# JanBeh/radiorust

Measured on NVIDIA B200. Metric: complex MS/s via FreqShift->Filter->Downsampler, higher is better.
Workload: dtype f32

## Files before the change

### radiorust_b200/csrc/rr_fused.cu

```cuda
#include <cuda.h>
#include <cuda_runtime.h>

#include <algorithm>
#include <cstdio>
#include <cstdlib>
#include <mutex>

#include "rr_kernels.h"
#include "rr_poly.cuh"
#include "rr_pk.cuh"

namespace rr {

namespace {

constexpr int FK = 512;
constexpr int FRK = 10;
constexpr int T_WARPS = FRK / 2;
constexpr int T_THREADS = 32 * T_WARPS;
constexpr int F_ROWS = 32;
constexpr int PITCH = FRK * 8;
constexpr int STAGE_ROWS = 528;
constexpr int STAGE_BYTES = STAGE_ROWS * PITCH;
constexpr int TW_UNITS = 17;
// ... 28 lines not shown
        : "memory");
}
__device__ __forceinline__ void mb_wait_long(uint32_t bar, uint32_t parity) {
    asm volatile(
        "{\n"
        ".reg .pred p;\n"
        "LWAIT_%=:\n"
        "mbarrier.try_wait.parity.acquire.cta.shared::cta.b64 p, [%0], %1, %2;\n"
        "@p bra LDONE_%=;\n"
        "bra LWAIT_%=;\n"
        "LDONE_%=:\n"
        "}\n" ::"r"(bar),
        "r"(parity), "r"(20000u)
        : "memory");
}
__device__ __forceinline__ pc f_lds(uint32_t addr) {
    pc r;
    asm volatile("ld.shared.v2.f32 {%0, %1}, [%2];" : "=f"(r.x), "=f"(r.y) : "r"(addr));
    return r;
}
__device__ __forceinline__ void f_lds2(uint32_t addr, pc& a, pc& b) {
    asm volatile("ld.shared.v4.f32 {%0, %1, %2, %3}, [%4];" : "=f"(a.x), "=f"(a.y), "=f"(b.x), "=f"(b.y) : "r"(addr));
}
__device__ __forceinline__ void f_sts(uint32_t addr, pc a) {
    asm volatile("st.shared.v2.f32 [%0], {%1, %2};" ::"r"(addr), "f"(a.x), "f"(a.y) : "memory");
}
__device__ __forceinline__ void f_sts2(uint32_t addr, pc a, pc b) {
    asm volatile("st.shared.v4.f32 [%0], {%1, %2, %3, %4};" ::"r"(addr), "f"(a.x), "f"(a.y), "f"(b.x), "f"(b.y) : "memory");
}
__device__ __forceinline__ void f_ldg2(const float4* p, pc& a, pc& b) {
    asm volatile("ld.global.nc.v4.f32 {%0, %1, %2, %3}, [%4];" : "=f"(a.x), "=f"(a.y), "=f"(b.x), "=f"(b.y) : "l"(p));
}

__device__ __forceinline__ pc f_rotation(uint32_t d, uint32_t numer_abs, uint32_t denom, double inv_m, int sign) {
    const uint32_t r = mulmod_fast(numer_abs, d % denom, denom, inv_m);
    double s, c;
    sincospi(2.0 * (double)r / (double)denom, &s, &c);
    return pc((float)c, (float)(sign < 0 ? -s : s));
}

__device__ __forceinline__ void f_pass1_store(pc (&v)[32], uint32_t tw_row, uint32_t xch_wr) {
    pdft_regs<32, +1>(v);
    pc w[3][2];
    f_lds2(tw_row, w[0][0], w[0][1]);
    f_lds2(tw_row + 16, w[1][0], w[1][1]);
#pragma unroll
    for (int m = 0; m < 16; ++m) {
        if (m + 2 < 16) f_lds2(tw_row + (m + 2) * 16, w[(m + 2) % 3][0], w[(m + 2) % 3][1]);
        f_sts(xch_wr + (2 * m) * PITCH, pcmul(v[2 * m], w[m % 3][0]));
        f_sts(xch_wr + (2 * m + 1) * PITCH, pcmul(v[2 * m + 1], w[m % 3][1]));
    }
}

#ifdef RR_FUSED_PROF
#define PROF(...) __VA_ARGS__
__device__ long long g_fused_prof[256 * 16];
#else
#define PROF(...)
#endif

struct FusedGeom {
    int steps, S0, hp, slot_bytes, slot_stride;
};
__host__ __device__ inline FusedGeom fused_geom(int P) {
    FusedGeom g;
    g.steps = P / 2;
    g.S0 = (g.steps + 1) / 2;
    g.hp = 2 * g.S0 + ((g.S0 & 1) ? 0 : 2);
    if (g.hp > P) g.hp = P;
    g.slot_bytes = F_ROWS * g.hp * 8;
    g.slot_stride = (g.slot_bytes + 127) / 128 * 128;
    return g;
}

template <int S_LO, int S_HI, bool HAS_NCO>
__device__ __forceinline__ void f_steps(pc (&acc)[FRK], const float4* __restrict__ xrow, const float4* __restrict__ crow, const float4* cf_base) {
#pragma unroll
    for (int st = S_LO; st < S_HI; ++st) {
        const float4 xv = xrow[st];
        pc x0(xv.x, xv.y), x1(xv.z, xv.w);
        if (HAS_NCO) {
            const float4 cv = crow[st];
            x0 = pcmul(x0, pc(cv.x, cv.y));
            x1 = pcmul(x1, pc(cv.z, cv.w));
        }
        const float4* cf = cf_base + st * 5;
        const float4 a0 = cf[0], a1 = cf[1], a2 = cf[2], a3 = cf[3], a4 = cf[4];
        const float k0[FRK] = {a0.x, a0.y, a0.z, a0.w, a1.x, a1.y, a1.z, a1.w, a2.x, a2.y};
        const float k1[FRK] = {a2.z, a2.w, a3.x, a3.y, a3.z, a3.w, a4.x, a4.y, a4.z, a4.w};
#pragma unroll
        for (int c = 0; c < FRK; ++c) {
            acc[c] = pfma_s(x0, k0[c], acc[c]);
            acc[c] = pfma_s(x1, k1[c], acc[c]);
        }
    }
}

}

template <int FW, int D, int NB, bool HAS_NCO, int PT>
__global__ void __launch_bounds__(T_THREADS + 32 * FW, 1)
k_fused(const __grid_constant__ CUtensorMap tmap, const FusedArgs a, const int n_streams) {
    extern __shared__ __align__(128) unsigned char smem[];
    const int warp = __shfl_sync(0xffffffffu, (int)(threadIdx.x >> 5), 0), lane = threadIdx.x & 31;
    const int P = PT > 0 ? PT : a.P;
    const FusedGeom geo = fused_geom(P);
    const int Lmax = a.Lmax, V = a.V, n_out = a.n_out;
    const int B = (n_out + V - 1) / V;
    const int n_tiles = (B * V + F_ROWS - 1) / F_ROWS;

    const int keep_bytes = ((Lmax * PITCH) + 127) / 128 * 128;
    unsigned char* const p_stage = smem;
    unsigned char* const p_tw = p_stage + 2 * STAGE_BYTES;
    unsigned char* const p_keep = p_tw + TW_BYTES;
    unsigned char* const p_ys = p_keep + keep_bytes;
    unsigned char* const p_ring = p_ys + (((size_t)NB * YS_STRIDE * 8 + 127) / 128 * 128);
    unsigned char* const p_colph = p_ring + (size_t)FW * D * geo.slot_stride;
    unsigned char* const p_bar = p_colph + (((size_t)FW * P * 8 + 127) / 128 * 128);
    const uint32_t bar_full = s_u32(p_bar), bar_empty = bar_full + 16, bar_ring = bar_full + 32;
    const uint32_t left_cnt = bar_ring + FW * D * 8;

    for (int e = threadIdx.x; e < 2 * STAGE_BYTES / 16; e += blockDim.x) reinterpret_cast<float4*>(p_stage)[e] = make_float4(0.f, 0.f, 0.f, 0.f);
    {
        const float2* __restrict__ twK = reinterpret_cast<const float2*>(a.twK);
        for (int e = threadIdx.x; e < FK; e += blockDim.x) {
            const int tr = e >> 5, k1 = e & 31;
            const float2 w = twK[(tr * k1) & (FK - 1)];
            const int off = (tr * TW_UNITS + (k1 >> 1)) * 16 + (k1 & 1) * 8;
            *reinterpret_cast<float2*>(p_tw + off) = w;
        }
    }
    if (threadIdx.x == 0) {
        asm volatile("prefetch.tensormap [%0];" ::"l"(&tmap) : "memory");
        mb_init(bar_full, FW);
        mb_init(bar_full + 8, FW);
        mb_init(bar_empty, T_WARPS);
        mb_init(bar_empty + 8, T_WARPS);
        for (int q = 0; q < FW * D; ++q) mb_init(bar_ring + q * 8, 1);
        asm volatile("st.shared.v2.u32 [%0], {%1, %1};" ::"r"(left_cnt), "r"(0u) : "memory");
        asm volatile("fence.mbarrier_init.release.cluster;" ::: "memory");
    }
    __syncthreads();

    const int n_my = (n_streams - (int)blockIdx.x + (int)gridDim.x - 1) / (int)gridDim.x;
    if (n_my <= 0) return;

    if (warp >= T_WARPS) {
        const int fw = warp - T_WARPS;
        const uint32_t ring_s = s_u32(p_ring) + fw * (D * geo.slot_stride);
        const uint32_t rbar = bar_ring + fw * (D * 8);
        float2* const colph = reinterpret_cast<float2*>(p_colph) + fw * P;
        const int steps = geo.steps, S0 = geo.S0, hp = geo.hp;
        const int half1_col0 = P - hp;
        const int J0 = (int)a.J0;
        const int hist_len = (int)(2 * a.n);
        const int hist_from = (int)a.hist_from;
        const int n_live = (n_out + F_ROWS - 1) / F_ROWS;
        const int rot_step = n_live % FW;
        auto tiles_from = [&](int j0) { return j0 < n_tiles ? (n_tiles - j0 + FW - 1) / FW : 0; };
        const int BV = B * V;
        const int tile_step = FW * F_ROWS;

        int i_so = 0, i_k = 0, i_half = 0, i_slot = 0;
        int i_j0 = fw, i_rot = 0, i_tw = tiles_from(fw);
        auto issue_next = [&]() {
            while (i_so < n_my) {
                if (i_k >= i_tw) {
                    ++i_so;
                    i_k = 0;
                    i_rot += rot_step;
                    if (i_rot >= FW) i_rot -= FW;
                    i_j0 = fw - i_rot + (fw < i_rot ? FW : 0);
                    i_tw = tiles_from(i_j0);
                    continue;
                }
                const int j = i_j0 + i_k * FW, half = i_half, so = i_so;
                i_half ^= 1;
                if (i_half == 0) ++i_k;
                const int rows_ok = min(F_ROWS, n_out - j * F_ROWS);
                if (rows_ok <= 0) continue;
                const int pos0 = j * (F_ROWS * P) - J0;
                const int coff = half ? half1_col0 : 0;
                const int sh = pos0 < 0 ? -1 : F_ROWS - rows_ok;
                if (lane == 0) {
                    mb_expect_tx(rbar + i_slot * 8, (uint32_t)geo.slot_bytes);
                    asm volatile("cp.async.bulk.tensor.3d.shared::cluster.global.mbarrier::complete_tx::bytes [%0], [%1, {%3, %4, %5}], [%2];" ::"r"(
                                     ring_s + i_slot * geo.slot_stride),
                                 "l"(&tmap), "r"(rbar + i_slot * 8), "r"(pos0 + coff - sh * P), "r"(sh), "r"((int)blockIdx.x + so * (int)gridDim.x)
                                 : "memory");
                }
                i_slot = (i_slot + 1 == D) ? 0 : i_slot + 1;
                return;
            }
        };
#pragma unroll 1
        for (int q = 0; q < D; ++q) issue_next();

        PROF(long long pr[8] = {0, 0, 0, 0, 0, 0, 0, 0}; const long long pr_t0 = clock64();)
        int c_slot = 0;
        uint32_t c_phase = 0;
        int gb_acq = -1;
        int gb_arr = -1;
        auto arrive_upto = [&](int gb_done) {
            for (int g2 = gb_arr + 1; g2 <= gb_done; ++g2) {
                while (gb_acq < g2) {
                    ++gb_acq;
                    mb_wait(bar_empty + (uint32_t)(gb_acq & 1) * 8, (uint32_t)(((gb_acq >> 1) & 1) ^ 1));
                }
                __syncwarp();
                if (lane == 0) mb_arrive(bar_full + (uint32_t)(g2 & 1) * 8);
            }
            if (gb_done > gb_arr) gb_arr = gb_done;
        };

        int rot = 0;
#pragma unroll 1
        for (int so = 0; so < n_my; ++so) {
            PROF(const long long pst0 = clock64();)
            const int s = (int)blockIdx.x + so * (int)gridDim.x;
            const int gb0 = so * B;
            const int j0 = fw - rot + (fw < rot ? FW : 0);
            const int tiles_w = tiles_from(j0);
            rot += rot_step;
            if (rot >= FW) rot -= FW;
            uint32_t denom = 1, numer_abs = 0, idx0 = 0;
            int sign = 0;
            float start = 0.f;
            pc rot_tile(1.f, 0.f);
            double inv_denom = 1.0;
            if (HAS_NCO && j0 < n_live) {
                const NcoStream ns = a.nco[s];
                denom = ns.denom;
                numer_abs = ns.numer_abs;
                sign = ns.sign;
                idx0 = ns.idx;
                start = (float)ns.start_phase;
                inv_denom = 1.0 / (double)denom;
                rot_tile = f_rotation((uint32_t)(tile_step * P), numer_abs, denom, inv_denom, sign);
                __syncwarp();
                for (int p = lane; p < P; p += 32) {
                    const pc c = f_rotation((uint32_t)p, numer_abs, denom, inv_denom, sign);
                    colph[p] = make_float2(c.x, c.y);
                }
                __syncwarp();
            }
            const float2* __restrict__ in = reinterpret_cast<const float2*>(a.in) + (long long)s * a.in_stride;
            const float2* __restrict__ hist_end = reinterpret_cast<const float2*>(a.hist2) + ((long long)s + 1) * hist_len;
            float2* __restrict__ hist_o = a.hist_out ? reinterpret_cast<float2*>(a.hist_out) + (long long)s * a.hist_stride : nullptr;
            float4* __restrict__ keep_o = reinterpret_cast<float4*>(reinterpret_cast<float2*>(a.ukeep_out) + (long long)s * a.ukeep_out_stride);
            const float4* cf_base = c_fcoef + a.coef_off4;
            const float4* __restrict__ crow = reinterpret_cast<const float4*>(colph);

            PROF(pr[7] += clock64() - pst0;)
            int blk = (j0 * F_ROWS) / V, off = (j0 * F_ROWS) - blk * V;
            pc rowph(1.f, 0.f);
#pragma unroll 1
            for (int k = 0; k < tiles_w; ++k) {
                const int r0 = (j0 + k * FW) * F_ROWS;
                const int row = r0 + lane;
                const int pos0 = r0 * P - J0;
                pc acc[FRK];
#pragma unroll
                for (int c = 0; c < FRK; ++c) acc[c] = pc(0.f, 0.f);
                PROF(long long pc0 = clock64();)
                if (r0 < n_out) {
                    if (HAS_NCO) {
                        if ((k & 15) == 0) {
                            const long long v = (long long)idx0 + pos0 + (long long)lane * P;
                            long long kk = v - (long long)floor((double)v * inv_denom) * (long long)denom;
                            if (kk < 0) kk += denom;
                            else if (kk >= (long long)denom) kk -= denom;
                            const cx<float> c = nco_phasor<float>(mulmod_fast(numer_abs, (uint32_t)kk, denom, inv_denom), denom, sign, start);
                            rowph = pc(c.x, c.y);
                        } else {
                            rowph = pcmul(rowph, rot_tile);
                        }
                    }
                    const int prow = pos0 + lane * P;
                    const bool to_hist = hist_o != nullptr && pos0 + F_ROWS * P > hist_from;
#pragma unroll 1
                    for (int half = 0; half < 2; ++half) {
                        const uint32_t slot_s = ring_s + c_slot * geo.slot_stride;
                        PROF(long long pw0 = clock64(); pr[0] += pw0 - pc0;)
                        mb_wait(rbar + c_slot * 8, c_phase);
                        PROF(long long pw1 = clock64(); pr[1] += pw1 - pw0;)
                        const int col0 = half ? half1_col0 : 0;
                        if (pos0 < 0) {
                            float2* dst = reinterpret_cast<float2*>(smem + (slot_s - s_u32(smem)));
                            const float r0x = __shfl_sync(0xffffffffu, rowph.x, 0), r0y = __shfl_sync(0xffffffffu, rowph.y, 0);
                            for (int cc = lane; cc < hp; cc += 32) {
                                const int p = col0 + cc;
                                const int pos = pos0 + p;
                                float2 q = make_float2(0.f, 0.f);
                                if (pos >= 0) {
                                    if (pos < (int)a.len) q = __ldg(in + pos);
                                } else if (pos >= -hist_len) {
                                    q = __ldg(hist_end + pos);
                                    if (HAS_NCO) {
                                        const float2 cph = colph[p];
                                        const pc y = pcmulc(pc(q.x, q.y), pcmul(pc(r0x, r0y), pc(cph.x, cph.y)));
                                        q = make_float2(y.x, y.y);
                                    }
                                }
                                dst[cc] = q;
                            }
                            __syncwarp();
                        }
                        const float4* __restrict__ xrow = reinterpret_cast<const float4*>(smem + (slot_s - s_u32(smem)) + lane * (hp * 8) - col0 * 8);
                        if (to_hist) {
                            const int st_lo = half ? S0 : 0, st_hi = half ? steps : S0;
#pragma unroll 2
                            for (int st = st_lo; st < st_hi; ++st) {
                                const float4 xv = xrow[st];
                                pc x0(xv.x, xv.y), x1(xv.z, xv.w);
                                if (HAS_NCO) {
                                    const float4 cv = crow[st];
                                    x0 = pcmul(x0, pc(cv.x, cv.y));
                                    x1 = pcmul(x1, pc(cv.z, cv.w));
                                }
                                const pc y0 = HAS_NCO ? pcmul(x0, rowph) : x0, y1 = HAS_NCO ? pcmul(x1, rowph) : x1;
                                const int jh = prow + 2 * st - hist_from;
                                if (row < n_out && jh >= -1) {
                                    if (jh >= 0) hist_o[jh] = make_float2(y0.x, y0.y);
                                    hist_o[jh + 1] = make_float2(y1.x, y1.y);
                                }
                                const float4* cf = cf_base + st * 5;
                                const float4 a0 = cf[0], a1 = cf[1], a2 = cf[2], a3 = cf[3], a4 = cf[4];
                                const float k0[FRK] = {a0.x, a0.y, a0.z, a0.w, a1.x, a1.y, a1.z, a1.w, a2.x, a2.y};
                                const float k1[FRK] = {a2.z, a2.w, a3.x, a3.y, a3.z, a3.w, a4.x, a4.y, a4.z, a4.w};
#pragma unroll
                                for (int c = 0; c < FRK; ++c) {
                                    acc[c] = pfma_s(x0, k0[c], acc[c]);
                                    acc[c] = pfma_s(x1, k1[c], acc[c]);
                                }
                            }
                        } else if constexpr (PT > 0) {
                            constexpr int STEPS_C = PT / 2, S0_C = (STEPS_C + 1) / 2;
                            if (half == 0) f_steps<0, S0_C, HAS_NCO>(acc, xrow, crow, cf_base);
                            else f_steps<S0_C, STEPS_C, HAS_NCO>(acc, xrow, crow, cf_base);
                        } else {
                            const int st_lo = half ? S0 : 0, st_hi = half ? steps : S0;
#pragma unroll 4
                            for (int st = st_lo; st < st_hi; ++st) {
                                const float4 xv = xrow[st];
                                pc x0(xv.x, xv.y), x1(xv.z, xv.w);
                                if (HAS_NCO) {
                                    const float4 cv = crow[st];
                                    x0 = pcmul(x0, pc(cv.x, cv.y));
                                    x1 = pcmul(x1, pc(cv.z, cv.w));
                                }
                                const float4* cf = cf_base + st * 5;
                                const float4 a0 = cf[0], a1 = cf[1], a2 = cf[2], a3 = cf[3], a4 = cf[4];
                                const float k0[FRK] = {a0.x, a0.y, a0.z, a0.w, a1.x, a1.y, a1.z, a1.w, a2.x, a2.y};
                                const float k1[FRK] = {a2.z, a2.w, a3.x, a3.y, a3.z, a3.w, a4.x, a4.y, a4.z, a4.w};
#pragma unroll
                                for (int c = 0; c < FRK; ++c) {
                                    acc[c] = pfma_s(x0, k0[c], acc[c]);
                                    acc[c] = pfma_s(x1, k1[c], acc[c]);
                                }
                            }
                        }
                        PROF(long long ps1 = clock64(); pr[2] += ps1 - pw1;)
                        asm volatile("fence.proxy.async.shared::cta;" ::: "memory");
                        __syncwarp();
                        PROF(long long ps2 = clock64(); pr[3] += ps2 - ps1;)
                        if (++c_slot == D) {
                            c_slot = 0;
                            c_phase ^= 1u;
                        }
                        issue_next();
                        PROF(pc0 = clock64(); pr[4] += pc0 - ps2;)
                    }
                }
                {
                    const int last_off = min(off + F_ROWS, BV - blk * V) - 1;
                    const int gb_hi = gb0 + blk + (last_off >= V ? 1 : 0);
                    PROF(long long pe0 = clock64(); pr[0] += pe0 - pc0;)
                    while (gb_acq < gb_hi) {
                        ++gb_acq;
                        mb_wait(bar_empty + (uint32_t)(gb_acq & 1) * 8, (uint32_t)(((gb_acq >> 1) & 1) ^ 1));
                    }
                    PROF(pc0 = clock64(); pr[5] += pc0 - pe0;)
                }
                if (row < BV) {
                    int b = blk, o = off + lane;
                    if (o >= V) {
                        o -= V;
                        ++b;
                    }
                    const uint32_t dst = s_u32(p_stage) + (uint32_t)((gb0 + b) & 1) * STAGE_BYTES + (Lmax + o) * PITCH;
                    const bool live = row < n_out;
                    const bool keep = live && row >= n_out - Lmax;
#pragma unroll
                    for (int c = 0; c < FRK; c += 2) {
                        pc y0 = acc[c], y1 = acc[c + 1];
                        if (HAS_NCO) {
                            y0 = pcmul(y0, rowph);
                            y1 = pcmul(y1, rowph);
                        }
                        if (!live) {
                            y0 = pc(0.f, 0.f);
                            y1 = pc(0.f, 0.f);
                        }
                        f_sts2(dst + c * 8, y0, y1);
                        if (keep) keep_o[((row - (n_out - Lmax)) * FRK + c) / 2] = make_float4(y0.x, y0.y, y1.x, y1.y);
                    }
                }
                __syncwarp();
                off += tile_step;
                while (off >= V) {
                    off -= V;
                    ++blk;
                }
                arrive_upto((k + 1 < tiles_w) ? gb0 + min(blk, B) - 1 : gb0 + B - 1);
                PROF(pr[6] += clock64() - pc0;)
            }
            if (tiles_w == 0) arrive_upto(gb0 + B - 1);
        }
        PROF(if (fw == 0 && lane == 0) {
            for (int q = 0; q < 7; ++q) g_fused_prof[blockIdx.x * 16 + q] = pr[q];
            g_fused_prof[blockIdx.x * 16 + 7] = pr[7];
            g_fused_prof[blockIdx.x * 16 + 8] = clock64() - pr_t0;
        })
        return;
    }

    const int tid = threadIdx.x;
    const int t = lane >> 1, gg = lane & 1;
    const int g = 2 * warp + gg;
    auto sync_t = [&]() { asm volatile("bar.sync 1, %0;" ::"n"(T_THREADS) : "memory"); };
    const uint32_t stage0 = s_u32(p_stage);
    const uint32_t tw_row = s_u32(p_tw) + t * (TW_UNITS * 16);
    const uint32_t tile_rd = t * PITCH + g * 8;
    const uint32_t xch_wr = 33 * t * PITCH + g * 8;
    const uint32_t xch_rd = t * PITCH + g * 8;
    const uint32_t keep_s = s_u32(p_keep) + warp * 16;
    float2* const ysave = reinterpret_cast<float2*>(p_ys);
    const float4* __restrict__ gtab = reinterpret_cast<const float4*>(a.gtab);
    const int hist_rows_per_lane = (Lmax + 31) / 32;

    const int n_blocks_total = n_my * B;
    auto copy_kept = [&](int so_k, int gb_k) {
        const uint32_t bytes = (uint32_t)(Lmax * PITCH), bar = bar_full + (uint32_t)(gb_k & 1) * 8;
        const float2* src = reinterpret_cast<const float2*>(a.ukeep_in) + (long long)((int)blockIdx.x + so_k * (int)gridDim.x) * a.ukeep_in_stride;
        asm volatile("fence.proxy.async.shared::cta;" ::: "memory");
        asm volatile("mbarrier.expect_tx.relaxed.cta.shared::cta.b64 [%0], %1;" ::"r"(bar), "r"(bytes) : "memory");
        asm volatile("cp.async.bulk.shared::cluster.global.mbarrier::complete_tx::bytes [%0], [%1], %2, [%3];" ::"r"(stage0 + (uint32_t)(gb_k & 1) * STAGE_BYTES),
                     "l"(src), "r"(bytes), "r"(bar)
                     : "memory");
    };
    if (tid == 0) {
        copy_kept(0, 0);
        if (B == 1 && n_my > 1) copy_kept(1, 1);
    }
    int parked = 0;
    int gb_first = 0;
    int so = 0, b = -1;
    PROF(long long tp[6] = {0, 0, 0, 0, 0, 0}; long long tc = clock64();)

#pragma unroll 1
    for (int gb = 0; gb < n_blocks_total; ++gb) {
        if (++b == B) {
            b = 0;
            ++so;
        }
        const int s = (int)blockIdx.x + so * (int)gridDim.x;
        const uint32_t stg = stage0 + (uint32_t)(gb & 1) * STAGE_BYTES;

        PROF({ long long n_ = clock64(); tp[0] += n_ - tc; tc = n_; })
        mb_wait_long(bar_full + (uint32_t)(gb & 1) * 8, (uint32_t)((gb >> 1) & 1));
        PROF({ long long n_ = clock64(); tp[1] += n_ - tc; tc = n_; })
#pragma unroll
        for (int q = 0; q < 12; ++q) {
            const int r = lane + 32 * q;
// ... 105 lines not shown
#pragma unroll
                        for (int k2 = 0; k2 < 16; ++k2) {
                            const int i = t + 16 * which + 32 * k2;
                            if (i >= Lmax && i < Lmax + V) {
                                const long long o = (long long)b_j * V + (i - Lmax);
                                if (o < n_out) {
                                    float2* dst = (out2 != nullptr && o >= a.out_split) ? out2 + (o - a.out_split) : out + o;
                                    *dst = make_float2(x[k2].x, -x[k2].y);
                                }
                            }
                        }
                    }
                }
                __syncwarp();
            }
            parked = 0;
            sync_t();
        }
        PROF({ long long n_ = clock64(); tp[4] += n_ - tc; tc = n_; })
        __syncwarp();
        if (lane == 0) {
            uint32_t left;
            asm volatile("atom.acq_rel.cta.shared::cta.add.u32 %0, [%1], 1;" : "=r"(left) : "r"(left_cnt + (uint32_t)(gb & 1) * 4) : "memory");
            if (left % T_WARPS == T_WARPS - 1) {
                int b2 = b + 2, so2 = so;
                while (b2 >= B) {
                    b2 -= B;
                    ++so2;
                }
                if (b2 == 0 && so2 < n_my) copy_kept(so2, gb + 2);
            }
            mb_arrive(bar_empty + (uint32_t)(gb & 1) * 8);
        }
    }
    PROF(if (tid == 0) for (int q = 0; q < 5; ++q) g_fused_prof[blockIdx.x * 16 + 9 + q] = tp[q];)
}

namespace {

using EncodeFn = CUresult (*)(CUtensorMap*, CUtensorMapDataType, cuuint32_t, void*, const cuuint64_t*, const cuuint64_t*, const cuuint32_t*,
                              const cuuint32_t*, CUtensorMapInterleave, CUtensorMapSwizzle, CUtensorMapL2promotion, CUtensorMapFloatOOBfill);
EncodeFn fused_encode_fn() {
    static EncodeFn fn = nullptr;
    static std::once_flag once;
    std::call_once(once, [] {
        void* p = nullptr;
        cudaDriverEntryPointQueryResult q;
        if (cudaGetDriverEntryPoint("cuTensorMapEncodeTiled", &p, cudaEnableDefault, &q) == cudaSuccess && q == cudaDriverEntryPointSuccess)
            fn = reinterpret_cast<EncodeFn>(p);
    });
    return fn;
}

template <int FW, int D, int NB> size_t fused_smem(int P, int Lmax) {
    const FusedGeom geo = fused_geom(P);
    size_t b = 2 * (size_t)STAGE_BYTES + TW_BYTES;
    b += ((size_t)Lmax * PITCH + 127) / 128 * 128;
    b += ((size_t)NB * YS_STRIDE * 8 + 127) / 128 * 128;
    b += (size_t)FW * D * geo.slot_stride;
    b += ((size_t)FW * P * 8 + 127) / 128 * 128;
    b += 32 + (size_t)FW * D * 8 + 64;
    return b;
}

template <int FW, int D, int NB>
cudaError_t launch_cfg(int n_streams, const FusedArgs& a, const CUtensorMap& tm, int sm_count, cudaStream_t st) {
    const size_t smem = fused_smem<FW, D, NB>(a.P, a.Lmax);
    if (smem > (size_t)227 * 1024) return cudaErrorInvalidConfiguration;
    const int grid = std::min(n_streams, sm_count);
    void (*kern)(const CUtensorMap, const FusedArgs, const int);
    switch (a.P) {
        case 50: kern = a.nco ? k_fused<FW, D, NB, true, 50> : k_fused<FW, D, NB, false, 50>; break;
        case 40: kern = a.nco ? k_fused<FW, D, NB, true, 40> : k_fused<FW, D, NB, false, 40>; break;
        case 20: kern = a.nco ? k_fused<FW, D, NB, true, 20> : k_fused<FW, D, NB, false, 20>; break;
        default: return cudaErrorNotSupported;
    }
    const cudaError_t e = cudaFuncSetAttribute(kern, cudaFuncAttributeMaxDynamicSharedMemorySize, (int)smem);
    if (e != cudaSuccess) return e;
    kern<<<grid, T_THREADS + 32 * FW, smem, st>>>(tm, a, n_streams);
#ifdef RR_FUSED_PROF
    static int calls = 0;
    static int at = std::getenv("RR_FUSED_PROF_CALL") ? std::atoi(std::getenv("RR_FUSED_PROF_CALL")) : 12;
    if (++calls == at) {
        cudaDeviceSynchronize();
        long long h[256 * 16];
        cudaMemcpyFromSymbol(h, g_fused_prof, sizeof h);
        for (int c : {0, 100})
            fprintf(stderr,
                    "cta %d n_out %d F0: tile-head %lld ring-wait %lld steps %lld fence+sync %lld issue %lld empty-wait %lld finalize %lld stream-setup %lld | total %lld"
                    " || T0: pre %lld wait-full %lld fwd+prod %lld sum+park %lld inverse %lld\n",
                    c, a.n_out, h[c * 16], h[c * 16 + 1], h[c * 16 + 2], h[c * 16 + 3], h[c * 16 + 4], h[c * 16 + 5], h[c * 16 + 6], h[c * 16 + 7], h[c * 16 + 8], h[c * 16 + 9],
                    h[c * 16 + 10], h[c * 16 + 11], h[c * 16 + 12], h[c * 16 + 13]);
    }
#endif
    return cudaGetLastError();
}

}

int fused_coef_slots() { return kFusedSlots; }

bool fused_supported(int rank_pad, long long P, int Lmax) {
    if (rank_pad != FRK || !(P == 50 || P == 40 || P == 20) || fused_encode_fn() == nullptr) return false;
    if (Lmax < 1 || FK - 1 - Lmax < 128 || Lmax > 383) return false;
    if ((P / 2) * 2 * FRK > kFusedSlotFloats) return false;
    return fused_smem<7, 2, 5>((int)P, Lmax) <= (size_t)227 * 1024;
}

cudaError_t fused_upload_coef(int slot, const float* acoef, int P, cudaStream_t st) {
    if (slot < 0 || slot >= kFusedSlots) return cudaErrorInvalidValue;
    const size_t n = (size_t)(P / 2) * 2 * FRK;
    if (n > (size_t)kFusedSlotFloats) return cudaErrorInvalidValue;
    return cudaMemcpyToSymbolAsync(c_fcoef, acoef, n * sizeof(float), (size_t)slot * kFusedSlotFloats * sizeof(float), cudaMemcpyHostToDevice, st);
}

cudaError_t launch_fused(int n_streams, const FusedArgs& a0, int sm_count, cudaStream_t st) {
    EncodeFn enc = fused_encode_fn();
    if (!enc) return cudaErrorNotSupported;
    FusedArgs a = a0;
    a.coef_off4 = a.coef_slot * (kFusedSlotFloats / 4);
    if ((uintptr_t)a.ukeep_in % 16 != 0 || (n_streams > 1 && a.ukeep_in_stride % 2 != 0)) return cudaErrorInvalidValue;
    const FusedGeom geo = fused_geom(a.P);
    CUtensorMap tm;
    const cuuint64_t dims[3] = {(cuuint64_t)a.len, (cuuint64_t)F_ROWS, (cuuint64_t)n_streams};
    const cuuint64_t sstride = n_streams > 1 ? (cuuint64_t)a.in_stride * 8 : (((cuuint64_t)a.len * 8 + 15) / 16) * 16;
    const cuuint64_t strides[2] = {(cuuint64_t)a.P * 8, sstride};
    const cuuint32_t box[3] = {(cuuint32_t)geo.hp, (cuuint32_t)F_ROWS, 1};
    const cuuint32_t estr[3] = {1, 1, 1};
    const CUresult r = enc(&tm, CU_TENSOR_MAP_DATA_TYPE_UINT64, 3, const_cast<void*>(a.in), dims, strides, box, estr, CU_TENSOR_MAP_INTERLEAVE_NONE,
                           CU_TENSOR_MAP_SWIZZLE_NONE, CU_TENSOR_MAP_L2_PROMOTION_L2_128B, CU_TENSOR_MAP_FLOAT_OOB_FILL_NONE);
    if (r != CUDA_SUCCESS) return cudaErrorInvalidValue;
    static int cfg = -1;
    if (cfg < 0) {
        cfg = 0;
        if (const char* e = std::getenv("RR_FUSED_CFG")) cfg = std::atoi(e);
    }
    switch (cfg) {
        case 1: return launch_cfg<6, 2, 8>(n_streams, a, tm, sm_count, st);
        default: return launch_cfg<7, 2, 5>(n_streams, a, tm, sm_count, st);
    }
}

}
```

Before: 529,200.

## Move polyphase filter accumulation onto tcgen05 TF32 MMA with split-precision operands

Replaces the per-thread FMA loop of the front-end filter with tcgen05 TF32 matrix multiplies. Input samples are split into hi and lo TF32 parts and written to TMEM, coefficients are pre-split into a shared-memory B matrix, and a dedicated MMA warp issues the products and signals completion through mbarriers. The epilogue is deferred by one round so staging overlaps the next MMA. Front-end warps drop from 7 to 4 (one per TMEM lane quadrant) and ring depth goes from 2 to 3. This adds TMEM allocation, extra synchronisation and split-precision error-compensation overhead.

Result: slower. 376,200 (median of 6 runs) (-28.9%).

```diff
diff --git a/radiorust_b200/csrc/rr_fused.cu b/radiorust_b200/csrc/rr_fused.cu
--- a/radiorust_b200/csrc/rr_fused.cu
+++ b/radiorust_b200/csrc/rr_fused.cu
@@ -104,6 +104,48 @@
     }
 }
 
+constexpr int MMA_N = 48;
+constexpr int MMA_NLO = 24;
+constexpr int MMA_M = 128;
+constexpr int TMEM_COLS = 512;
+__host__ __device__ constexpr int mma_k(int P) { return (2 * P + 7) / 8 * 8; }
+constexpr uint32_t B_LBO = (MMA_N / 8) * 128;
+constexpr uint32_t B_SBO = 128;
+__host__ __device__ constexpr int bmat_bytes(int P) { return mma_k(P) * MMA_N * 4; }
+constexpr uint32_t MMA_IDESC = (1u << 4) | (2u << 7) | (2u << 10) | ((uint32_t)(MMA_N >> 3) << 17) | ((uint32_t)(MMA_M >> 4) << 24);
+
+__device__ __forceinline__ uint32_t tf32_rn(float x) { return (__float_as_uint(x) + 0x1000u) & 0xffffe000u; }
+
+__device__ __forceinline__ uint64_t smem_desc(uint32_t saddr) {
+    return (uint64_t)((saddr & 0x3FFFFu) >> 4) | ((uint64_t)(B_LBO >> 4) << 16) | ((uint64_t)(B_SBO >> 4) << 32) | (1ull << 46);
+}
+__device__ __forceinline__ void tc_fence_before() { asm volatile("tcgen05.fence::before_thread_sync;" ::: "memory"); }
+__device__ __forceinline__ void tc_fence_after() { asm volatile("tcgen05.fence::after_thread_sync;" ::: "memory"); }
+__device__ __forceinline__ void tm_st4(uint32_t ta, const uint32_t* v) {
+    asm volatile("tcgen05.st.sync.aligned.32x32b.x4.b32 [%0], {%1, %2, %3, %4};" ::"r"(ta), "r"(v[0]), "r"(v[1]), "r"(v[2]), "r"(v[3]) : "memory");
+}
+__device__ __forceinline__ void tm_st8(uint32_t ta, const uint32_t* v) {
+    asm volatile("tcgen05.st.sync.aligned.32x32b.x8.b32 [%0], {%1, %2, %3, %4, %5, %6, %7, %8};" ::"r"(ta), "r"(v[0]), "r"(v[1]), "r"(v[2]), "r"(v[3]),
+                 "r"(v[4]), "r"(v[5]), "r"(v[6]), "r"(v[7])
+                 : "memory");
+}
+__device__ __forceinline__ void tm_st16(uint32_t ta, const uint32_t* v) {
+    asm volatile("tcgen05.st.sync.aligned.32x32b.x16.b32 [%0], {%1, %2, %3, %4, %5, %6, %7, %8, %9, %10, %11, %12, %13, %14, %15, %16};" ::"r"(ta),
+                 "r"(v[0]), "r"(v[1]), "r"(v[2]), "r"(v[3]), "r"(v[4]), "r"(v[5]), "r"(v[6]), "r"(v[7]), "r"(v[8]), "r"(v[9]), "r"(v[10]), "r"(v[11]),
+                 "r"(v[12]), "r"(v[13]), "r"(v[14]), "r"(v[15])
+                 : "memory");
+}
+__device__ __forceinline__ void tm_ld4(uint32_t ta, uint32_t* v) {
+    asm volatile("tcgen05.ld.sync.aligned.32x32b.x4.b32 {%0, %1, %2, %3}, [%4];" : "=r"(v[0]), "=r"(v[1]), "=r"(v[2]), "=r"(v[3]) : "r"(ta) : "memory");
+}
+__device__ __forceinline__ void tm_ld16(uint32_t ta, uint32_t* v) {
+    asm volatile("tcgen05.ld.sync.aligned.32x32b.x16.b32 {%0, %1, %2, %3, %4, %5, %6, %7, %8, %9, %10, %11, %12, %13, %14, %15}, [%16];"
+                 : "=r"(v[0]), "=r"(v[1]), "=r"(v[2]), "=r"(v[3]), "=r"(v[4]), "=r"(v[5]), "=r"(v[6]), "=r"(v[7]), "=r"(v[8]), "=r"(v[9]), "=r"(v[10]),
+                   "=r"(v[11]), "=r"(v[12]), "=r"(v[13]), "=r"(v[14]), "=r"(v[15])
+                 : "r"(ta)
+                 : "memory");
+}
+
 #ifdef RR_FUSED_PROF
 #define PROF(...) __VA_ARGS__
 __device__ long long g_fused_prof[256 * 16];
@@ -125,41 +167,73 @@
     return g;
 }
 
-template <int S_LO, int S_HI, bool HAS_NCO>
-__device__ __forceinline__ void f_steps(pc (&acc)[FRK], const float4* __restrict__ xrow, const float4* __restrict__ crow, const float4* cf_base) {
-#pragma unroll
-    for (int st = S_LO; st < S_HI; ++st) {
-        const float4 xv = xrow[st];
-        pc x0(xv.x, xv.y), x1(xv.z, xv.w);
-        if (HAS_NCO) {
-            const float4 cv = crow[st];
-            x0 = pcmul(x0, pc(cv.x, cv.y));
-            x1 = pcmul(x1, pc(cv.z, cv.w));
-        }
-        const float4* cf = cf_base + st * 5;
-        const float4 a0 = cf[0], a1 = cf[1], a2 = cf[2], a3 = cf[3], a4 = cf[4];
-        const float k0[FRK] = {a0.x, a0.y, a0.z, a0.w, a1.x, a1.y, a1.z, a1.w, a2.x, a2.y};
-        const float k1[FRK] = {a2.z, a2.w, a3.x, a3.y, a3.z, a3.w, a4.x, a4.y, a4.z, a4.w};
-#pragma unroll
-        for (int c = 0; c < FRK; ++c) {
-            acc[c] = pfma_s(x0, k0[c], acc[c]);
-            acc[c] = pfma_s(x1, k1[c], acc[c]);
-        }
+template <int S_LO, int S_HI, int KP, bool HAS_NCO, bool TO_HIST>
+__device__ __forceinline__ void f_split(const float4* __restrict__ xrow, const float4* __restrict__ crow, uint32_t ta, pc rowph, float2* hist_o,
+                                        int jh0, bool row_ok) {
+    if constexpr (S_LO < S_HI) {
+        constexpr int NS = S_HI - S_LO < 4 ? S_HI - S_LO : 4;
+        uint32_t hi[4 * NS], lo[4 * NS];
+#pragma unroll
+        for (int i = 0; i < NS; ++i) {
+            const int st = S_LO + i;
+            const float4 xv = xrow[st];
+            pc x0(xv.x, xv.y), x1(xv.z, xv.w);
+            if (HAS_NCO) {
+                const float4 cv = crow[st];
+                x0 = pcmul(x0, pc(cv.x, cv.y));
+                x1 = pcmul(x1, pc(cv.z, cv.w));
+            }
+            if (TO_HIST) {
+                const pc y0 = HAS_NCO ? pcmul(x0, rowph) : x0, y1 = HAS_NCO ? pcmul(x1, rowph) : x1;
+                const int jh = jh0 + 2 * st;
+                if (row_ok && jh >= -1) {
+                    if (jh >= 0) hist_o[jh] = make_float2(y0.x, y0.y);
+                    hist_o[jh + 1] = make_float2(y1.x, y1.y);
+                }
+            }
+            const float v[4] = {x0.x, x0.y, x1.x, x1.y};
+#pragma unroll
+            for (int e = 0; e < 4; ++e) {
+                hi[4 * i + e] = tf32_rn(v[e]);
+                lo[4 * i + e] = tf32_rn(v[e] - __uint_as_float(hi[4 * i + e]));
+            }
+        }
+        const uint32_t c0 = ta + 4 * S_LO;
+        if constexpr (NS == 4) {
+            tm_st16(c0, hi);
+            tm_st16(c0 + KP, lo);
+        } else {
+            if constexpr (NS >= 2) {
+                tm_st8(c0, hi);
+                tm_st8(c0 + KP, lo);
+            }
+            if constexpr (NS & 1) {
+                tm_st4(c0 + 4 * (NS - 1), hi + 4 * (NS - 1));
+                tm_st4(c0 + KP + 4 * (NS - 1), lo + 4 * (NS - 1));
+            }
+        }
+        f_split<S_LO + NS, S_HI, KP, HAS_NCO, TO_HIST>(xrow, crow, ta, rowph, hist_o, jh0, row_ok);
     }
 }
 
 }
 
 template <int FW, int D, int NB, bool HAS_NCO, int PT>
-__global__ void __launch_bounds__(T_THREADS + 32 * FW, 1)
+__global__ void __launch_bounds__(T_THREADS + 32 * FW + 32, 1)
 k_fused(const __grid_constant__ CUtensorMap tmap, const FusedArgs a, const int n_streams) {
+    static_assert(FW == 4, "one front-end warp per TMEM lane quadrant: the four tiles of a round fill the M = 128 rows");
+    constexpr int P = PT;
+    constexpr int KP = mma_k(P);
+    static_assert(4 * KP + 2 * MMA_N <= TMEM_COLS, "two A buffers (hi | lo) and two D buffers in the TMEM allocation");
     extern __shared__ __align__(128) unsigned char smem[];
     const int warp = __shfl_sync(0xffffffffu, (int)(threadIdx.x >> 5), 0), lane = threadIdx.x & 31;
-    const int P = PT > 0 ? PT : a.P;
     const FusedGeom geo = fused_geom(P);
     const int Lmax = a.Lmax, V = a.V, n_out = a.n_out;
     const int B = (n_out + V - 1) / V;
     const int n_tiles = (B * V + F_ROWS - 1) / F_ROWS;
+    const int n_my = (n_streams - (int)blockIdx.x + (int)gridDim.x - 1) / (int)gridDim.x;
+    if (n_my <= 0) return;
+    const int MMA_WARP = T_WARPS + FW;
 
     const int keep_bytes = ((Lmax * PITCH) + 127) / 128 * 128;
     unsigned char* const p_stage = smem;
@@ -168,9 +242,13 @@
     unsigned char* const p_ys = p_keep + keep_bytes;
     unsigned char* const p_ring = p_ys + (((size_t)NB * YS_STRIDE * 8 + 127) / 128 * 128);
     unsigned char* const p_colph = p_ring + (size_t)FW * D * geo.slot_stride;
-    unsigned char* const p_bar = p_colph + (((size_t)FW * P * 8 + 127) / 128 * 128);
-    const uint32_t bar_full = s_u32(p_bar), bar_empty = bar_full + 16, bar_ring = bar_full + 32;
+    unsigned char* const p_bmat = p_colph + (((size_t)FW * P * 8 + 127) / 128 * 128);
+    unsigned char* const p_bar = p_bmat + bmat_bytes(P);
+    const uint32_t bar_full = s_u32(p_bar), bar_empty = bar_full + 16;
+    const uint32_t bar_afull = bar_full + 32, bar_dready = bar_full + 48;
+    const uint32_t bar_ring = bar_full + 64;
     const uint32_t left_cnt = bar_ring + FW * D * 8;
+    const uint32_t tmem_slot = left_cnt + 8;
 
     for (int e = threadIdx.x; e < 2 * STAGE_BYTES / 16; e += blockDim.x) reinterpret_cast<float4*>(p_stage)[e] = make_float4(0.f, 0.f, 0.f, 0.f);
     {
@@ -182,36 +260,113 @@
             *reinterpret_cast<float2*>(p_tw + off) = w;
         }
     }
+    {
+        const float* __restrict__ cf = reinterpret_cast<const float*>(c_fcoef) + a.coef_off4 * 4;
+        for (int e = threadIdx.x; e < KP * MMA_N; e += blockDim.x) {
+            const int k = e / MMA_N, n = e - k * MMA_N;
+            const int p = k >> 1, nn = n < MMA_NLO ? n : n - MMA_NLO, c = nn >> 1;
+            float v = 0.f;
+            if (p < P && c < FRK && (nn & 1) == (k & 1)) {
+                const float av = cf[(p >> 1) * 2 * FRK + (p & 1) * FRK + c];
+                const float hi = __uint_as_float(tf32_rn(av));
+                v = n < MMA_NLO ? hi : __uint_as_float(tf32_rn(av - hi));
+            }
+            *reinterpret_cast<float*>(p_bmat + (k >> 2) * B_LBO + (n >> 3) * B_SBO + (n & 7) * 16 + (k & 3) * 4) = v;
+        }
+        asm volatile("fence.proxy.async.shared::cta;" ::: "memory");
+    }
     if (threadIdx.x == 0) {
         asm volatile("prefetch.tensormap [%0];" ::"l"(&tmap) : "memory");
         mb_init(bar_full, FW);
         mb_init(bar_full + 8, FW);
         mb_init(bar_empty, T_WARPS);
         mb_init(bar_empty + 8, T_WARPS);
+        mb_init(bar_afull, FW);
+        mb_init(bar_afull + 8, FW);
+        mb_init(bar_dready, 1);
+        mb_init(bar_dready + 8, 1);
         for (int q = 0; q < FW * D; ++q) mb_init(bar_ring + q * 8, 1);
         asm volatile("st.shared.v2.u32 [%0], {%1, %1};" ::"r"(left_cnt), "r"(0u) : "memory");
         asm volatile("fence.mbarrier_init.release.cluster;" ::: "memory");
     }
+    if (warp == MMA_WARP) {
+        asm volatile("tcgen05.alloc.cta_group::1.sync.aligned.shared::cta.b32 [%0], %1;" ::"r"(tmem_slot), "n"(TMEM_COLS) : "memory");
+        asm volatile("tcgen05.relinquish_alloc_permit.cta_group::1.sync.aligned;" ::: "memory");
+    }
+    tc_fence_before();
     __syncthreads();
-
-    const int n_my = (n_streams - (int)blockIdx.x + (int)gridDim.x - 1) / (int)gridDim.x;
-    if (n_my <= 0) return;
+    tc_fence_after();
+
+    const int n_live = (n_out + F_ROWS - 1) / F_ROWS;
+    const int rot_step = n_tiles % FW;
+    auto tiles_from = [&](int j0) { return j0 < n_tiles ? (n_tiles - j0 + FW - 1) / FW : 0; };
+    auto n_rounds = [&]() {
+        int R = 0;
+        for (int f = 0; f < FW; ++f) {
+            int cnt = 0, rot = 0;
+            for (int so = 0; so < n_my; ++so) {
+                cnt += tiles_from(f - rot + (f < rot ? FW : 0));
+                rot += rot_step;
+                if (rot >= FW) rot -= FW;
+            }
+            R = max(R, cnt);
+        }
+        return R;
+    };
+
+    if (warp == MMA_WARP) {
+        const uint32_t tmem = *reinterpret_cast<volatile uint32_t*>(smem + (tmem_slot - s_u32(smem)));
+        const uint64_t bdesc = smem_desc(s_u32(p_bmat));
+        const int R = n_rounds();
+#pragma unroll 1
+        for (int r = 0; r < R; ++r) {
+            mb_wait(bar_afull + (uint32_t)(r & 1) * 8, (uint32_t)((r >> 1) & 1));
+            tc_fence_after();
+            if (lane == 0) {
+                const uint32_t ta = tmem + (uint32_t)(r & 1) * (2 * KP), td = tmem + 4 * KP + (uint32_t)(r & 1) * MMA_N;
+#pragma unroll
+                for (int pass = 0; pass < 2; ++pass) {
+#pragma unroll
+                    for (int s = 0; s < KP / 8; ++s) {
+                        asm volatile(
+                            "{\n.reg .pred p;\nsetp.ne.b32 p, %4, 0;\n"
+                            "tcgen05.mma.cta_group::1.kind::tf32 [%0], [%1], %2, %3, p;\n}\n" ::"r"(td),
+                            "r"(ta + pass * KP + 8 * s), "l"(bdesc + (uint64_t)((s * 2 * B_LBO) >> 4)), "r"(MMA_IDESC), "r"(pass | s)
+                            : "memory");
+                    }
+                }
+                asm volatile("tcgen05.commit.cta_group::1.mbarrier::arrive::one.shared::cluster.b64 [%0];" ::"r"(bar_dready + (uint32_t)(r & 1) * 8) : "memory");
+            }
+            __syncwarp();
+        }
+        asm volatile("bar.sync 2, %0;" ::"n"(32 * (FW + 1)) : "memory");
+        tc_fence_after();
+        asm volatile("tcgen05.dealloc.cta_group::1.sync.aligned.b32 %0, %1;" ::"r"(tmem), "n"(TMEM_COLS) : "memory");
+        return;
+    }
 
     if (warp >= T_WARPS) {
         const int fw = warp - T_WARPS;
+        const uint32_t tmem = *reinterpret_cast<volatile uint32_t*>(smem + (tmem_slot - s_u32(smem)));
+        const uint32_t tm_row = tmem + ((uint32_t)(warp & 3) * 32 << 16);
         const uint32_t ring_s = s_u32(p_ring) + fw * (D * geo.slot_stride);
         const uint32_t rbar = bar_ring + fw * (D * 8);
         float2* const colph = reinterpret_cast<float2*>(p_colph) + fw * P;
-        const int steps = geo.steps, S0 = geo.S0, hp = geo.hp;
+        constexpr int steps = P / 2, S0 = (steps + 1) / 2;
+        const int hp = geo.hp;
         const int half1_col0 = P - hp;
         const int J0 = (int)a.J0;
         const int hist_len = (int)(2 * a.n);
         const int hist_from = (int)a.hist_from;
-        const int n_live = (n_out + F_ROWS - 1) / F_ROWS;
-        const int rot_step = n_live % FW;
-        auto tiles_from = [&](int j0) { return j0 < n_tiles ? (n_tiles - j0 + FW - 1) / FW : 0; };
         const int BV = B * V;
         const int tile_step = FW * F_ROWS;
+        const int R = n_rounds();
+
+        for (int col = 2 * P; col < KP; ++col) {
+            const uint32_t z = 0u;
+#pragma unroll
+            for (int q = 0; q < 4; ++q) asm volatile("tcgen05.st.sync.aligned.32x32b.x1.b32 [%0], {%1};" ::"r"(tm_row + q * KP + col), "r"(z) : "memory");
+        }
 
         int i_so = 0, i_k = 0, i_half = 0, i_slot = 0;
         int i_j0 = fw, i_rot = 0, i_tw = tiles_from(fw);
@@ -248,7 +403,7 @@
 #pragma unroll 1
         for (int q = 0; q < D; ++q) issue_next();
 
-        PROF(long long pr[8] = {0, 0, 0, 0, 0, 0, 0, 0}; const long long pr_t0 = clock64();)
+        PROF(long long pr[8] = {0, 0, 0, 0, 0, 0, 0, 0}; const long long pr_t0 = clock64(); long long pc0 = pr_t0;)
         int c_slot = 0;
         uint32_t c_phase = 0;
         int gb_acq = -1;
@@ -263,6 +418,87 @@
                 if (lane == 0) mb_arrive(bar_full + (uint32_t)(g2 & 1) * 8);
             }
             if (gb_done > gb_arr) gb_arr = gb_done;
+        };
+
+        int rnd = 0;
+        bool p_tile = false;
+        int p_r0 = 0, p_blk = 0, p_off = 0, p_so = 0;
+        pc p_rowph(1.f, 0.f);
+        int owed = -1;
+        auto finish = [&]() {
+            const int r = rnd - 1;
+            PROF(long long pd0 = clock64();)
+            mb_wait(bar_dready + (uint32_t)(r & 1) * 8, (uint32_t)((r >> 1) & 1));
+            tc_fence_after();
+            PROF(long long pd1 = clock64(); pr[3] += pd1 - pd0;)
+            if (p_tile) {
+                pc acc[FRK];
+#pragma unroll
+                for (int c = 0; c < FRK; ++c) acc[c] = pc(0.f, 0.f);
+                if (p_r0 < n_out) {
+                    const uint32_t td = tm_row + 4 * KP + (uint32_t)(r & 1) * MMA_N;
+                    uint32_t d[2 * MMA_NLO];
+                    tm_ld16(td, d);
+                    tm_ld4(td + 16, d + 16);
+                    tm_ld16(td + MMA_NLO, d + MMA_NLO);
+                    tm_ld4(td + MMA_NLO + 16, d + MMA_NLO + 16);
+                    asm volatile("tcgen05.wait::ld.sync.aligned;" ::: "memory");
+#pragma unroll
+                    for (int c = 0; c < FRK; ++c)
+                        acc[c] = pc(__uint_as_float(d[2 * c]) + __uint_as_float(d[MMA_NLO + 2 * c]),
+                                    __uint_as_float(d[2 * c + 1]) + __uint_as_float(d[MMA_NLO + 2 * c + 1]));
+                }
+                tc_fence_before();
+                const int last_off = min(p_off + F_ROWS, BV - p_blk * V) - 1;
+                const int p_gb0 = p_so * B;
+                const int gb_hi = p_gb0 + p_blk + (last_off >= V ? 1 : 0);
+                PROF(long long pe0 = clock64(); pr[5] += pe0 - pd1;)
+                while (gb_acq < gb_hi) {
+                    ++gb_acq;
+                    mb_wait(bar_empty + (uint32_t)(gb_acq & 1) * 8, (uint32_t)(((gb_acq >> 1) & 1) ^ 1));
+                }
+                PROF(pd1 = clock64(); pr[4] += pd1 - pe0;)
+                const int row = p_r0 + lane;
+                if (row < BV) {
+                    int b = p_blk, o = p_off + lane;
+                    if (o >= V) {
+                        o -= V;
+                        ++b;
+                    }
+                    const uint32_t dst = s_u32(p_stage) + (uint32_t)((p_gb0 + b) & 1) * STAGE_BYTES + (Lmax + o) * PITCH;
+                    const bool live = row < n_out;
+                    const bool keep = live && row >= n_out - Lmax;
+#pragma unroll
+                    for (int c = 0; c < FRK; c += 2) {
+                        pc y0 = acc[c], y1 = acc[c + 1];
+                        if (HAS_NCO) {
+                            y0 = pcmul(y0, p_rowph);
+                            y1 = pcmul(y1, p_rowph);
+                        }
+                        if (!live) {
+                            y0 = pc(0.f, 0.f);
+                            y1 = pc(0.f, 0.f);
+                        }
+                        f_sts2(dst + c * 8, y0, y1);
+                        if (keep) {
+                            float4* keep_o = reinterpret_cast<float4*>(reinterpret_cast<float2*>(a.ukeep_out) +
+                                                                       (long long)((int)blockIdx.x + p_so * (int)gridDim.x) * a.ukeep_out_stride);
+                            keep_o[((row - (n_out - Lmax)) * FRK + c) / 2] = make_float4(y0.x, y0.y, y1.x, y1.y);
+                        }
+                    }
+                }
+                __syncwarp();
+                PROF(pr[5] += clock64() - pd1;)
+            }
+            arrive_upto(owed);
+        };
+        auto end_round = [&]() {
+            asm volatile("tcgen05.wait::st.sync.aligned;" ::: "memory");
+            tc_fence_before();
+            __syncwarp();
+            if (lane == 0) mb_arrive(bar_afull + (uint32_t)(rnd & 1) * 8);
+            if (rnd > 0) finish();
+            ++rnd;
         };
 
         int rot = 0;
@@ -299,11 +535,9 @@
             const float2* __restrict__ in = reinterpret_cast<const float2*>(a.in) + (long long)s * a.in_stride;
             const float2* __restrict__ hist_end = reinterpret_cast<const float2*>(a.hist2) + ((long long)s + 1) * hist_len;
             float2* __restrict__ hist_o = a.hist_out ? reinterpret_cast<float2*>(a.hist_out) + (long long)s * a.hist_stride : nullptr;
-            float4* __restrict__ keep_o = reinterpret_cast<float4*>(reinterpret_cast<float2*>(a.ukeep_out) + (long long)s * a.ukeep_out_stride);
-            const float4* cf_base = c_fcoef + a.coef_off4;
             const float4* __restrict__ crow = reinterpret_cast<const float4*>(colph);
 
-            PROF(pr[7] += clock64() - pst0;)
+            PROF(pr[6] += clock64() - pst0;)
             int blk = (j0 * F_ROWS) / V, off = (j0 * F_ROWS) - blk * V;
             pc rowph(1.f, 0.f);
 #pragma unroll 1
@@ -311,10 +545,6 @@
                 const int r0 = (j0 + k * FW) * F_ROWS;
                 const int row = r0 + lane;
                 const int pos0 = r0 * P - J0;
-                pc acc[FRK];
-#pragma unroll
-                for (int c = 0; c < FRK; ++c) acc[c] = pc(0.f, 0.f);
-                PROF(long long pc0 = clock64();)
                 if (r0 < n_out) {
                     if (HAS_NCO) {
                         if ((k & 15) == 0) {
@@ -328,14 +558,14 @@
                             rowph = pcmul(rowph, rot_tile);
                         }
                     }
-                    const int prow = pos0 + lane * P;
+                    const int jh0 = pos0 + lane * P - hist_from;
                     const bool to_hist = hist_o != nullptr && pos0 + F_ROWS * P > hist_from;
 #pragma unroll 1
                     for (int half = 0; half < 2; ++half) {
                         const uint32_t slot_s = ring_s + c_slot * geo.slot_stride;
-                        PROF(long long pw0 = clock64(); pr[0] += pw0 - pc0;)
+                        PROF(long long pw0 = clock64(); pr[7] += pw0 - pc0;)
                         mb_wait(rbar + c_slot * 8, c_phase);
-                        PROF(long long pw1 = clock64(); pr[1] += pw1 - pw0;)
+                        PROF(long long pw1 = clock64(); pr[0] += pw1 - pw0;)
                         const int col0 = half ? half1_col0 : 0;
                         if (pos0 < 0) {
                             float2* dst = reinterpret_cast<float2*>(smem + (slot_s - s_u32(smem)));
@@ -359,119 +589,51 @@
                             __syncwarp();
                         }
                         const float4* __restrict__ xrow = reinterpret_cast<const float4*>(smem + (slot_s - s_u32(smem)) + lane * (hp * 8) - col0 * 8);
+                        const uint32_t ta = tm_row + (uint32_t)(rnd & 1) * (2 * KP);
                         if (to_hist) {
-                            const int st_lo = half ? S0 : 0, st_hi = half ? steps : S0;
-#pragma unroll 2
-                            for (int st = st_lo; st < st_hi; ++st) {
-                                const float4 xv = xrow[st];
-                                pc x0(xv.x, xv.y), x1(xv.z, xv.w);
-                                if (HAS_NCO) {
-                                    const float4 cv = crow[st];
-                                    x0 = pcmul(x0, pc(cv.x, cv.y));
-                                    x1 = pcmul(x1, pc(cv.z, cv.w));
-                                }
-                                const pc y0 = HAS_NCO ? pcmul(x0, rowph) : x0, y1 = HAS_NCO ? pcmul(x1, rowph) : x1;
-                                const int jh = prow + 2 * st - hist_from;
-                                if (row < n_out && jh >= -1) {
-                                    if (jh >= 0) hist_o[jh] = make_float2(y0.x, y0.y);
-                                    hist_o[jh + 1] = make_float2(y1.x, y1.y);
-                                }
-                                const float4* cf = cf_base + st * 5;
-                                const float4 a0 = cf[0], a1 = cf[1], a2 = cf[2], a3 = cf[3], a4 = cf[4];
-                                const float k0[FRK] = {a0.x, a0.y, a0.z, a0.w, a1.x, a1.y, a1.z, a1.w, a2.x, a2.y};
-                                const float k1[FRK] = {a2.z, a2.w, a3.x, a3.y, a3.z, a3.w, a4.x, a4.y, a4.z, a4.w};
-#pragma unroll
-                                for (int c = 0; c < FRK; ++c) {
-                                    acc[c] = pfma_s(x0, k0[c], acc[c]);
-                                    acc[c] = pfma_s(x1, k1[c], acc[c]);
-                                }
-                            }
-                        } else if constexpr (PT > 0) {
-                            constexpr int STEPS_C = PT / 2, S0_C = (STEPS_C + 1) / 2;
-                            if (half == 0) f_steps<0, S0_C, HAS_NCO>(acc, xrow, crow, cf_base);
-                            else f_steps<S0_C, STEPS_C, HAS_NCO>(acc, xrow, crow, cf_base);
+                            if (half == 0) f_split<0, S0, KP, HAS_NCO, true>(xrow, crow, ta, rowph, hist_o, jh0, row < n_out);
+                            else f_split<S0, steps, KP, HAS_NCO, true>(xrow, crow, ta, rowph, hist_o, jh0, row < n_out);
                         } else {
-                            const int st_lo = half ? S0 : 0, st_hi = half ? steps : S0;
-#pragma unroll 4
-                            for (int st = st_lo; st < st_hi; ++st) {
-                                const float4 xv = xrow[st];
-                                pc x0(xv.x, xv.y), x1(xv.z, xv.w);
-                                if (HAS_NCO) {
-                                    const float4 cv = crow[st];
-                                    x0 = pcmul(x0, pc(cv.x, cv.y));
-                                    x1 = pcmul(x1, pc(cv.z, cv.w));
-                                }
-                                const float4* cf = cf_base + st * 5;
-                                const float4 a0 = cf[0], a1 = cf[1], a2 = cf[2], a3 = cf[3], a4 = cf[4];
-                                const float k0[FRK] = {a0.x, a0.y, a0.z, a0.w, a1.x, a1.y, a1.z, a1.w, a2.x, a2.y};
-                                const float k1[FRK] = {a2.z, a2.w, a3.x, a3.y, a3.z, a3.w, a4.x, a4.y, a4.z, a4.w};
-#pragma unroll
-                                for (int c = 0; c < FRK; ++c) {
-                                    acc[c] = pfma_s(x0, k0[c], acc[c]);
-                                    acc[c] = pfma_s(x1, k1[c], acc[c]);
-                                }
-                            }
+                            if (half == 0) f_split<0, S0, KP, HAS_NCO, false>(xrow, crow, ta, rowph, nullptr, 0, false);
+                            else f_split<S0, steps, KP, HAS_NCO, false>(xrow, crow, ta, rowph, nullptr, 0, false);
                         }
-                        PROF(long long ps1 = clock64(); pr[2] += ps1 - pw1;)
+                        PROF(long long ps1 = clock64(); pr[1] += ps1 - pw1;)
                         asm volatile("fence.proxy.async.shared::cta;" ::: "memory");
                         __syncwarp();
-                        PROF(long long ps2 = clock64(); pr[3] += ps2 - ps1;)
                         if (++c_slot == D) {
                             c_slot = 0;
                             c_phase ^= 1u;
                         }
                         issue_next();
-                        PROF(pc0 = clock64(); pr[4] += pc0 - ps2;)
+                        PROF(pc0 = clock64(); pr[2] += pc0 - ps1;)
                     }
                 }
-                {
-                    const int last_off = min(off + F_ROWS, BV - blk * V) - 1;
-                    const int gb_hi = gb0 + blk + (last_off >= V ? 1 : 0);
-                    PROF(long long pe0 = clock64(); pr[0] += pe0 - pc0;)
-                    while (gb_acq < gb_hi) {
-                        ++gb_acq;
-                        mb_wait(bar_empty + (uint32_t)(gb_acq & 1) * 8, (uint32_t)(((gb_acq >> 1) & 1) ^ 1));
-                    }
-                    PROF(pc0 = clock64(); pr[5] += pc0 - pe0;)
-                }
-                if (row < BV) {
-                    int b = blk, o = off + lane;
-                    if (o >= V) {
-                        o -= V;
-                        ++b;
-                    }
-                    const uint32_t dst = s_u32(p_stage) + (uint32_t)((gb0 + b) & 1) * STAGE_BYTES + (Lmax + o) * PITCH;
-                    const bool live = row < n_out;
-                    const bool keep = live && row >= n_out - Lmax;
-#pragma unroll
-                    for (int c = 0; c < FRK; c += 2) {
-                        pc y0 = acc[c], y1 = acc[c + 1];
-                        if (HAS_NCO) {
-                            y0 = pcmul(y0, rowph);
-                            y1 = pcmul(y1, rowph);
-                        }
-                        if (!live) {
-                            y0 = pc(0.f, 0.f);
-                            y1 = pc(0.f, 0.f);
-                        }
-                        f_sts2(dst + c * 8, y0, y1);
-                        if (keep) keep_o[((row - (n_out - Lmax)) * FRK + c) / 2] = make_float4(y0.x, y0.y, y1.x, y1.y);
-                    }
-                }
-                __syncwarp();
+                end_round();
+                PROF(pc0 = clock64();)
+                p_tile = true;
+                p_r0 = r0;
+                p_blk = blk;
+                p_off = off;
+                p_so = so;
+                p_rowph = rowph;
                 off += tile_step;
                 while (off >= V) {
                     off -= V;
                     ++blk;
                 }
-                arrive_upto((k + 1 < tiles_w) ? gb0 + min(blk, B) - 1 : gb0 + B - 1);
-                PROF(pr[6] += clock64() - pc0;)
-            }
-            if (tiles_w == 0) arrive_upto(gb0 + B - 1);
-        }
+                owed = max(owed, (k + 1 < tiles_w) ? gb0 + min(blk, B) - 1 : gb0 + B - 1);
+            }
+            if (tiles_w == 0) owed = max(owed, gb0 + B - 1);
+        }
+        while (rnd < R) {
+            end_round();
+            p_tile = false;
+        }
+        if (rnd > 0) finish();
+        tc_fence_before();
+        asm volatile("bar.arrive 2, %0;" ::"n"(32 * (FW + 1)) : "memory");
         PROF(if (fw == 0 && lane == 0) {
-            for (int q = 0; q < 7; ++q) g_fused_prof[blockIdx.x * 16 + q] = pr[q];
-            g_fused_prof[blockIdx.x * 16 + 7] = pr[7];
+            for (int q = 0; q < 8; ++q) g_fused_prof[blockIdx.x * 16 + q] = pr[q];
             g_fused_prof[blockIdx.x * 16 + 8] = clock64() - pr_t0;
         })
         return;
@@ -683,20 +845,23 @@
     return fn;
 }
 
-template <int FW, int D, int NB> size_t fused_smem(int P, int Lmax) {
+constexpr int FUSED_FW = 4, FUSED_D = 3, FUSED_NB = 5;
+
+size_t fused_smem(int P, int Lmax) {
     const FusedGeom geo = fused_geom(P);
     size_t b = 2 * (size_t)STAGE_BYTES + TW_BYTES;
     b += ((size_t)Lmax * PITCH + 127) / 128 * 128;
-    b += ((size_t)NB * YS_STRIDE * 8 + 127) / 128 * 128;
-    b += (size_t)FW * D * geo.slot_stride;
-    b += ((size_t)FW * P * 8 + 127) / 128 * 128;
-    b += 32 + (size_t)FW * D * 8 + 64;
+    b += ((size_t)FUSED_NB * YS_STRIDE * 8 + 127) / 128 * 128;
+    b += (size_t)FUSED_FW * FUSED_D * geo.slot_stride;
+    b += ((size_t)FUSED_FW * P * 8 + 127) / 128 * 128;
+    b += (size_t)bmat_bytes(P);
+    b += 64 + (size_t)FUSED_FW * FUSED_D * 8 + 16;
     return b;
 }
 
-template <int FW, int D, int NB>
 cudaError_t launch_cfg(int n_streams, const FusedArgs& a, const CUtensorMap& tm, int sm_count, cudaStream_t st) {
-    const size_t smem = fused_smem<FW, D, NB>(a.P, a.Lmax);
+    constexpr int FW = FUSED_FW, D = FUSED_D, NB = FUSED_NB;
+    const size_t smem = fused_smem(a.P, a.Lmax);
     if (smem > (size_t)227 * 1024) return cudaErrorInvalidConfiguration;
     const int grid = std::min(n_streams, sm_count);
     void (*kern)(const CUtensorMap, const FusedArgs, const int);
@@ -708,7 +873,7 @@
     }
     const cudaError_t e = cudaFuncSetAttribute(kern, cudaFuncAttributeMaxDynamicSharedMemorySize, (int)smem);
     if (e != cudaSuccess) return e;
-    kern<<<grid, T_THREADS + 32 * FW, smem, st>>>(tm, a, n_streams);
+    kern<<<grid, T_THREADS + 32 * FW + 32, smem, st>>>(tm, a, n_streams);
 #ifdef RR_FUSED_PROF
     static int calls = 0;
     static int at = std::getenv("RR_FUSED_PROF_CALL") ? std::atoi(std::getenv("RR_FUSED_PROF_CALL")) : 12;
@@ -718,7 +883,7 @@
         cudaMemcpyFromSymbol(h, g_fused_prof, sizeof h);
         for (int c : {0, 100})
             fprintf(stderr,
-                    "cta %d n_out %d F0: tile-head %lld ring-wait %lld steps %lld fence+sync %lld issue %lld empty-wait %lld finalize %lld stream-setup %lld | total %lld"
+                    "cta %d n_out %d F0: ring-wait %lld split+sttm %lld fence+issue %lld d-wait %lld empty-wait %lld epilogue %lld stream-setup %lld tile-head %lld | total %lld"
                     " || T0: pre %lld wait-full %lld fwd+prod %lld sum+park %lld inverse %lld\n",
                     c, a.n_out, h[c * 16], h[c * 16 + 1], h[c * 16 + 2], h[c * 16 + 3], h[c * 16 + 4], h[c * 16 + 5], h[c * 16 + 6], h[c * 16 + 7], h[c * 16 + 8], h[c * 16 + 9],
                     h[c * 16 + 10], h[c * 16 + 11], h[c * 16 + 12], h[c * 16 + 13]);
@@ -735,7 +900,7 @@
     if (rank_pad != FRK || !(P == 50 || P == 40 || P == 20) || fused_encode_fn() == nullptr) return false;
     if (Lmax < 1 || FK - 1 - Lmax < 128 || Lmax > 383) return false;
     if ((P / 2) * 2 * FRK > kFusedSlotFloats) return false;
-    return fused_smem<7, 2, 5>((int)P, Lmax) <= (size_t)227 * 1024;
+    return fused_smem((int)P, Lmax) <= (size_t)227 * 1024;
 }
 
 cudaError_t fused_upload_coef(int slot, const float* acoef, int P, cudaStream_t st) {
@@ -761,15 +926,7 @@
     const CUresult r = enc(&tm, CU_TENSOR_MAP_DATA_TYPE_UINT64, 3, const_cast<void*>(a.in), dims, strides, box, estr, CU_TENSOR_MAP_INTERLEAVE_NONE,
                            CU_TENSOR_MAP_SWIZZLE_NONE, CU_TENSOR_MAP_L2_PROMOTION_L2_128B, CU_TENSOR_MAP_FLOAT_OOB_FILL_NONE);
     if (r != CUDA_SUCCESS) return cudaErrorInvalidValue;
-    static int cfg = -1;
-    if (cfg < 0) {
-        cfg = 0;
-        if (const char* e = std::getenv("RR_FUSED_CFG")) cfg = std::atoi(e);
-    }
-    switch (cfg) {
-        case 1: return launch_cfg<6, 2, 8>(n_streams, a, tm, sm_count, st);
-        default: return launch_cfg<7, 2, 5>(n_streams, a, tm, sm_count, st);
-    }
-}
-
-}
+    return launch_cfg(n_streams, a, tm, sm_count, st);
+}
+
+}
```
